# amd/aocl-sparse

Measured on AMD Instinct MI355X. Metric: CSR SpMV fp64 GFLOP/s + achieved-HBM-GB/s %roofline, higher is better.
Workload: dtype f64; 1 GPU; aoclsparse_dmv, 5-pt Laplacian grid 4096x4096 (m=16777216, nnz=83869696), alpha=1 beta=0; BASELINE configs[1] scaled past the 256 MiB Infinity Cache; parallelism=replicas x1, device=AMD Radeon Graphics (gfx950:sramecc+:...

## Files before the change

### aocl-sparse_amd/__init__.py

```python
import ctypes
import os
from ctypes import POINTER, byref, c_bool, c_char_p, c_double, c_float, c_int, c_int32, c_void_p

_HERE = os.path.dirname(os.path.abspath(__file__))
LIB_PATH = os.environ.get("AOCLSPARSE_MI355_LIB") or os.path.join(_HERE, "lib", "libaoclsparse_mi355.so")
INCLUDE_DIR = os.path.join(os.path.dirname(_HERE), "include")

OP_NONE, OP_TRANSPOSE, OP_CONJ_TRANSPOSE = 111, 112, 113
BASE_ZERO, BASE_ONE = 0, 1
TYPE_GENERAL, TYPE_SYMMETRIC, TYPE_HERMITIAN, TYPE_TRIANGULAR = 0, 1, 2, 3
DIAG_NON_UNIT, DIAG_UNIT, DIAG_ZERO = 0, 1, 2
FILL_LOWER, FILL_UPPER = 0, 1
ORDER_ROW, ORDER_COLUMN = 0, 1
STAGE_NNZ_COUNT, STAGE_FINALIZE, STAGE_FULL = 0, 1, 2
MEM_MINIMAL, MEM_UNRESTRICTED = 0, 1
PTR_AUTO, PTR_HOST, PTR_DEVICE = 0, 1, 2
OPTION_SPMV_KERNEL, OPTION_SELL, OPTION_SPMV_STRICT, OPTION_ALTERNATE_SWEEPS, OPTION_TRSV_CHUNKS = 0, 1, 2, 3, 4
OPTION_SELL_VALUES = 5
OPTION_ILU_SEARCH = 16
ILU_SEARCH_MIN = 21
COO_KEEP, COO_SUM = 0, 1
COO_KEEP_MAP = 16
COO_SORT_TILE = 4096
ORDER_SHORT_MAX = 32
ORDER_LDS_MAX = 2048
CLEAN_ROW_WAVE = 64

STATUS = {
    0: "success", 1: "not_implemented", 2: "invalid_pointer", 3: "invalid_size", 4: "internal_error",
    5: "invalid_value", 6: "invalid_index_value", 7: "maxit", 8: "user_stop", 9: "wrong_type",
    10: "memory_error", 11: "numerical_error", 12: "invalid_operation", 13: "unsorted_input",
    14: "invalid_kid",
}
# ... 414 lines not shown
    "aoclsparse_mi355_replicas_cloned": (c_int, [_P]),
    "aoclsparse_mi355_scsrmm_multi": (c_int, [c_int, c_float, _P, _P, c_int, _P, _I, _I, c_float, _P, _I, _I, _P]),
    "aoclsparse_mi355_dcsrmm_multi_slabs": (c_int, [c_int, c_double, _P, _P, c_int, _P, _I, _I, c_double, _P, _I, _I, _P]),
    "aoclsparse_mi355_scsrmm_shard": (c_int, [c_int, c_float, _P, _P, c_int, _P, _I, _I, c_float, _P, _I, _I, _I]),
    "aoclsparse_mi355_export_diag": (c_int, [_P, POINTER(_P), POINTER(_P), POINTER(_I)]),
    "aoclsparse_mi355_get_spmv_info": (c_int, [_P, c_int, POINTER(SpmvInfo)]),
    "aoclsparse_mi355_get_sell_values": (c_int, [_P, c_int, POINTER(_I)]),
    "aoclsparse_mi355_get_sell_packing": (c_int, [_P, c_int, POINTER(_I), POINTER(_I), POINTER(_I)]),
    "aoclsparse_mi355_get_sell_records": (c_int, [_P, c_int, POINTER(_I), POINTER(_I)]),
    "aoclsparse_mi355_get_sell_period": (c_int, [_P, c_int, POINTER(_I), POINTER(_I), POINTER(_I), POINTER(_I)]),
    "aoclsparse_mi355_sell_find_period": (c_int, [_I, _P, _P, _I, POINTER(_I), POINTER(ctypes.c_longlong)]),
    "aoclsparse_mi355_get_sell_march": (c_int, [_P, c_int, POINTER(_I), POINTER(_I), POINTER(_I), POINTER(_I)]),
    "aoclsparse_mi355_get_sell_keep_info": (c_int, [_P, c_int, _P]),
    "aoclsparse_mi355_sell_find_march": (c_int, [_I, _P, _P, POINTER(_I), _I, POINTER(_I)]),
    "aoclsparse_mi355_sell_march_rule": (c_int, [_I, _I, POINTER(_I), _I, _I, _I, _I, POINTER(_I)]),
    "aoclsparse_mi355_get_trsv_levels": (c_int, [_P, c_int, c_int, POINTER(_I)]),
    "aoclsparse_mi355_get_trsv_info": (c_int, [_P, c_int, c_int, POINTER(TrsvInfo)]),
    "aoclsparse_mi355_trsv_status": (c_int, [_P]),
    "aoclsparse_mi355_set_trsv_schedule": (c_int, [_I]),
    "aoclsparse_mi355_set_csrmm_beta0_overwrite": (c_int, [c_int]),
    "aoclsparse_mi355_invalidate": (c_int, [_P]),
    "aoclsparse_mi355_release_staging": (c_int, [POINTER(ctypes.c_size_t)]),
    "mi355_csrmv_plan_bound": (_I, [_I, _I]),
    "mi355_csrmv_plan_host": (_I, [_I, _I, _I, _P, _P]),
    "mi355_sell_slice_records": (_I, [_I, _P, _P, ctypes.c_longlong, _P]),
    "mi355_dcsrmv": (c_int, [_P, _I, _I, _I, _I, c_double, _I, _P, _P, _P, _P, _I, _P, c_double, _P]),
    "mi355_scsrmv": (c_int, [_P, _I, _I, _I, _I, c_float, _I, _P, _P, _P, _P, _I, _P, c_float, _P]),
    "mi355_dcsrmm": (c_int, [_P, _I, _I, c_double, _I, _I, _P, _P, _P, _P, _I, _I, c_double, _P, _I]),
}

# ... 268 lines not shown
    def sell_packing(self, op=OP_NONE):
        b, w, u = _I(-1), _I(-1), _I(-1)
        assert lib().aoclsparse_mi355_get_sell_packing(self.h, op, byref(b), byref(w), byref(u)) == 0
        return b.value, w.value, u.value

    def sell_records(self, op=OP_NONE):
        u, e = _I(-1), _I(-1)
        assert lib().aoclsparse_mi355_get_sell_records(self.h, op, byref(u), byref(e)) == 0
        return u.value, e.value

    def sell_period(self, op=OP_NONE):
        a, b, p, c = _I(-1), _I(-1), _I(-1), _I(-1)
        assert lib().aoclsparse_mi355_get_sell_period(self.h, op, byref(a), byref(b), byref(p), byref(c)) == 0
        return a.value, b.value, p.value, c.value

    def sell_march(self, op=OP_NONE):
        a, b, g, c = _I(-1), _I(-1), _I(-1), _I(-1)
        assert lib().aoclsparse_mi355_get_sell_march(self.h, op, byref(a), byref(b), byref(g), byref(c)) == 0
        return a.value, b.value, g.value, c.value

    def sell_keep_info(self, op=OP_NONE):
        info = SellKeepInfo(struct_size=ctypes.sizeof(SellKeepInfo))
        st = lib().aoclsparse_mi355_get_sell_keep_info(self.h, op, byref(info))
        assert st == 0, STATUS.get(st, st)
        return info

    def trsv_info(self, fill, op=OP_NONE):
        info = TrsvInfo()
        assert lib().aoclsparse_mi355_get_trsv_info(self.h, fill, op, byref(info)) == 0
        return info
# ... 167 lines not shown
    assert records.ndim == 2 and records.shape[1] == 4 and lists.shape == (records.shape[0], 8)
    out = (_I * 2)(-1, -1)
    st = lib().aoclsparse_mi355_sell_find_march(records.shape[0], _ptr(records), _ptr(lists), (_I * 4)(*rng), word_bytes, out)
    assert st == 0, STATUS.get(st, st)
    return tuple(out)


def sell_march_rule(nslices, max_width, rng, stack, alias_map, value_bytes=8, slices_per_wavefront=2):
    out = (_I * 4)(-1, -1, -1, -1)
    st = lib().aoclsparse_mi355_sell_march_rule(nslices, max_width, (_I * 4)(*rng), stack, alias_map, value_bytes,
                                                slices_per_wavefront, out)
    assert st == 0, STATUS.get(st, st)
    return tuple(out)


def device_info():
    dev, cus = c_int32(-1), c_int32(0)
    name = ctypes.create_string_buffer(256)
    st = lib().aoclsparse_mi355_device_info(byref(dev), byref(cus), name)
    return st, dev.value, cus.value, name.value.decode()


def hip_runtime_path():
    buf = ctypes.create_string_buffer(4096)
    st = lib().aoclsparse_mi355_hip_runtime_path(buf, 4096)
    return st, buf.value.decode()


def timer_start():
    return lib().aoclsparse_mi355_timer_start()
# ... 48 lines not shown
```

### aocl-sparse_amd/csrc/internal.hpp

```cpp
#pragma once

#include "aoclsparse.h"
#include "aoclsparse_mi355.h"

#include <hip/hip_runtime_api.h>

#include <atomic>
#include <algorithm>
#include <thread>
#include <cstdlib>
#include <cstdio>
#include <chrono>
#include <cstddef>
#include <cstdint>
#include <cstdint>
#include <exception>
#include <memory>
#include <mutex>
#include <functional>
#include <new>
#include <shared_mutex>
#include <system_error>
#include <vector>

// ... 1235 lines not shown
aoclsparse_status launch_roti(hipStream_t s, aoclsparse_int nnz, T *x, const aoclsparse_int *indx, T *y, T c, T sn);
template <typename T>
aoclsparse_status launch_doti(hipStream_t s, aoclsparse_int nnz, const T *x, const aoclsparse_int *indx, const T *y,
                              bool conj, T *partial, T *out);

template <typename T>
aoclsparse_status launch_sorv_level(hipStream_t s, const aoclsparse_int *rows, aoclsparse_int count, int base,
                                    const aoclsparse_int *ptr, const aoclsparse_int *ind, const T *val, T omega, T *x,
                                    const T *xold, const T *b);

constexpr int SPMV_TREE_MIN = 32;
constexpr int spmv_maxrows(int tile)
{
    return tile / 2 < 512 ? tile / 2 : 512;
}

}
```

### aocl-sparse_amd/csrc/matrix.cpp

```cpp
#include "spg_host.hpp"

#include <algorithm>
#include <atomic>
#include <climits>
#include <cstdlib>
#include <cstring>
#include <numeric>
#include <thread>

using namespace mi355;

namespace mi355
{

doid get_doid(const _aoclsparse_mat_descr *d, aoclsparse_operation op)
{
    const bool tr = op != aoclsparse_operation_none;
    switch(d->type)
    {
    case aoclsparse_matrix_type_general:
        return tr ? doid::gt : doid::gn;
    case aoclsparse_matrix_type_symmetric:
    case aoclsparse_matrix_type_hermitian:
        return d->fill_mode == aoclsparse_fill_mode_lower ? doid::sl : doid::su;
// ... 446 lines not shown
    }
    blocks[2 * nb]     = m;
    blocks[2 * nb + 1] = row_ptr[m] - base;
    if(long_rows)
        *long_rows = lr;
    if(max_row)
        *max_row = mx;
    return nb;
}

static aoclsparse_int choose_tile(aoclsparse_int , aoclsparse_int nnz, size_t vsize)
{
    if(vsize == 4 && (long long)nnz >= 1024LL * 256 * 16)
        return 2048;
    static const bool xcd_order = getenv("AOCLSPARSE_MI355_SPMV_XCD_ORDER") && getenv("AOCLSPARSE_MI355_SPMV_XCD_ORDER")[0] == '1';
    return ((long long)nnz < 1024LL * 256 * 16 ? 512 : 1024) | (xcd_order ? 1 : 0);
}

static void plan_rows_range(aoclsparse_int r0, aoclsparse_int r1, aoclsparse_index_base base, aoclsparse_int tile,
                            const aoclsparse_int *row_ptr, std::vector<aoclsparse_int> &out, aoclsparse_int &lr,
                            aoclsparse_int &mx)
{
    aoclsparse_int i = r0;
    while(i < r1)
    {
        const aoclsparse_int start = row_ptr[i] - base;
        aoclsparse_int       j     = i;
        while(j < r1 && j - i < spmv_maxrows(tile) && (row_ptr[j + 1] - base) - start <= tile)
            j++;
        if(j == i)
// ... 1292 lines not shown
```

### aocl-sparse_amd/csrc/runtime.cpp

```cpp
#include "internal.hpp"

#include <dlfcn.h>
#include <sys/mman.h>

#include <cctype>
#include <condition_variable>
#include <cstdio>
#include <cstdlib>
#include <cstring>
#include <thread>

#include <sched.h>

namespace mi355
{

aoclsparse_status map_hip_error(hipError_t e)
{
    if(e == hipSuccess)
        return aoclsparse_status_success;
    (void)hipGetLastError();
    if(e == hipErrorOutOfMemory)
        return aoclsparse_status_memory_error;
    return aoclsparse_status_internal_error;
// ... 275 lines not shown
}

std::atomic<bool> &csrmm_beta0_overwrite_flag()
{
    static std::atomic<bool> flag{[] {
        const char *e = std::getenv("AOCLSPARSE_MI355_CSRMM_BETA0_OVERWRITE");
        return e && std::atoi(e) != 0;
    }()};
    return flag;
}

namespace
{
    std::atomic<int> g_plan_options[aoclsparse_mi355_option_count] = {{0}, {-1}, {0}, {1}, {-1}, {-1}};
    std::atomic<int> g_ilu_search{-1};
}
unsigned long long stream_uid(hipStream_t s)
{
    using get_id_t = hipError_t (*)(hipStream_t, unsigned long long *);
    static const get_id_t get_id = [] {
        Dl_info info;
        if(!dladdr(reinterpret_cast<const void *>(&hipStreamCreate), &info) || !info.dli_fname)
            return static_cast<get_id_t>(nullptr);
        void *h = dlopen(info.dli_fname, RTLD_LAZY | RTLD_NOLOAD);
        return h ? reinterpret_cast<get_id_t>(dlsym(h, "hipStreamGetId")) : static_cast<get_id_t>(nullptr);
    }();
    unsigned long long id = 0;
    if(!get_id)
        return 0;
    if(get_id(s, &id) != hipSuccess)
    {
        (void)hipGetLastError();
        id = 0;
    }
    return id;
}

int plan_option(aoclsparse_mi355_option option)
{
    if(option == aoclsparse_mi355_option_ilu_search)
        return g_ilu_search.load(std::memory_order_relaxed);
    return option >= 0 && option < aoclsparse_mi355_option_count ? g_plan_options[option].load(std::memory_order_relaxed) : 0;
}

bool csrmm_reads_c(bool beta_nonzero)
{
    return beta_nonzero || !csrmm_beta0_overwrite_flag().load(std::memory_order_relaxed);
}

bool Runtime::is_device_pointer(const void *p)
{
    if(tl_device_scope > 0)
        return true;
    if(pointer_mode == aoclsparse_mi355_pointer_device)
        return true;
    if(pointer_mode == aoclsparse_mi355_pointer_host)
// ... 70 lines not shown
        if(scope.status == aoclsparse_status_success)
            f += r->release_staging();
    }
    if(bytes_freed)
        *bytes_freed = f;
    return aoclsparse_status_success;
}

aoclsparse_status aoclsparse_mi355_set_option(aoclsparse_mi355_option option, aoclsparse_int value)
{
    if(option == aoclsparse_mi355_option_ilu_search)
    {
        if(value < -1 || value > 1)
            return aoclsparse_status_invalid_value;
        g_ilu_search.store((int)value, std::memory_order_relaxed);
        return aoclsparse_status_success;
    }
    if(option < 0 || option >= aoclsparse_mi355_option_count)
        return aoclsparse_status_invalid_value;
    if(option == aoclsparse_mi355_option_spmv_kernel && (value < 0 || value > 2))
        return aoclsparse_status_invalid_value;
    if(option == aoclsparse_mi355_option_sell && (value < -1 || value > 1))
        return aoclsparse_status_invalid_value;
    if(option == aoclsparse_mi355_option_spmv_strict && (value < 0 || value > 1))
        return aoclsparse_status_invalid_value;
    if(option == aoclsparse_mi355_option_alternate_sweeps && (value < 0 || value > 1))
        return aoclsparse_status_invalid_value;
    if(option == aoclsparse_mi355_option_trsv_chunks && (value < -1 || value > 1))
        return aoclsparse_status_invalid_value;
    if(option == aoclsparse_mi355_option_sell_values && (value < -1 || value > 1))
// ... 181 lines not shown
```

### aocl-sparse_amd/csrc/spmv_api.cpp

```cpp
#include "internal.hpp"

#include <algorithm>
#include <cstring>
#include <vector>

using namespace mi355;

namespace
{

inline bool valid_op(aoclsparse_operation op)
{
    return op == aoclsparse_operation_none || op == aoclsparse_operation_transpose
           || op == aoclsparse_operation_conjugate_transpose;
}
inline bool valid_base(int b)
{
    return b == aoclsparse_index_base_zero || b == aoclsparse_index_base_one;
}
inline bool valid_type(int t)
{
    return t >= aoclsparse_matrix_type_general && t <= aoclsparse_matrix_type_triangular;
}

// ... 238 lines not shown
        }
    }
    std::shared_lock<std::shared_mutex> r(A->guard);
    return run_on_device_csr<T>(cs, kid, *dcsr, *plan, *alpha, x, *beta, y, dcsr->n, dcsr->m);
}

struct RawPlan
{
    const void               *key = nullptr;
    aoclsparse_int            m = -1, nnz = -1, base = -1;
    std::shared_ptr<SpmvPlan> plan;
};
constexpr int RAW_CACHE = 8;
RawPlan       g_raw[RAW_CACHE];
int           g_raw_next = 0;

template <typename T>
aoclsparse_status csrmv_t(aoclsparse_operation trans, const T *alpha, aoclsparse_int m,
                          aoclsparse_int n, aoclsparse_int nnz, const T *val,
                          const aoclsparse_int *col, const aoclsparse_int *row,
                          const aoclsparse_mat_descr descr, const T *x, const T *beta, T *y,
                          aoclsparse_matrix_data_type vt)
{
    if(!alpha || !beta)
        return aoclsparse_status_invalid_pointer;
    if(!descr)
        return aoclsparse_status_invalid_pointer;
    if(!valid_base(descr->base))
        return aoclsparse_status_invalid_value;
    if(!valid_type(descr->type))
// ... 153 lines not shown
                        held = e.plan;
            }
            if(rt.plan_stale_host && *rt.plan_stale_host)
            {
                std::lock_guard<std::mutex> g(rt.lock);
                *rt.plan_stale_host = 0;
                for(auto &e : g_raw)
                    e = RawPlan();
                held.reset();
            }
            if(held && !rt.plan_stale_dev)
                held.reset();
            if(!held)
            {
                fresh_plan = true;
                std::vector<aoclsparse_int> hrow((size_t)m + 1);
                MI355_HIP_TRY(hipMemcpy(hrow.data(), row, sizeof(aoclsparse_int) * ((size_t)m + 1),
                                        hipMemcpyDeviceToHost));
                held = std::make_shared<SpmvPlan>();
                st   = build_spmv_plan(m, nnz, descr->base, hrow.data(), *held, sizeof(T));
                if(st != aoclsparse_status_success)
                    return st;
                std::lock_guard<std::mutex> g(rt.lock);
                RawPlan                    *slot = nullptr;
                for(auto &e : g_raw)
                    if(e.key == row && e.m == m && e.nnz == nnz && e.base == descr->base)
                        slot = &e;
                if(!slot)
                {
                    slot       = &g_raw[g_raw_next];
// ... 154 lines not shown
            break;
        }
    int  order  = 0;
    bool strict = false;
    if(A->val_type == aoclsparse_smat)
        resolve_order<float>(kid, d.m, d.nnz, p.max_row_nnz, order, strict);
    else
        resolve_order<double>(kid, d.m, d.nnz, p.max_row_nnz, order, strict);
    info->order = order;
    if(plan_option(aoclsparse_mi355_option_spmv_strict) == 1)
        strict = true;
    info->tree_min = ((info->kernel == 1 || info->kernel == 2) && order == 0 && !strict) ? SPMV_TREE_MIN : 0;
    return aoclsparse_status_success;
}

aoclsparse_status aoclsparse_mi355_get_sell_values(const aoclsparse_matrix A, aoclsparse_operation op, aoclsparse_int *table_entries)
{
    if(!A || !table_entries)
        return aoclsparse_status_invalid_pointer;
    std::shared_lock<std::shared_mutex> r(A->guard);
    const SpmvPlan                     &p = op != aoclsparse_operation_none ? A->plan_trans : A->plan_user;
    *table_entries                        = p.sell.valid ? p.sell.ntab : 0;
    return aoclsparse_status_success;
}

aoclsparse_status aoclsparse_mi355_get_sell_packing(const aoclsparse_matrix A, aoclsparse_operation op, aoclsparse_int *index_bits,
                                                    aoclsparse_int *word_bytes, aoclsparse_int *uniform_slices)
{
    if(!A || !index_bits || !word_bytes || !uniform_slices)
        return aoclsparse_status_invalid_pointer;
// ... 110 lines not shown
```

### aocl-sparse_amd/csrc/spmv_kernels.hip

```cpp
#include "internal.hpp"

#include <hip/hip_runtime.h>

#include <cstdio>
#include <cstdlib>
#include <vector>

#include <algorithm>

namespace mi355
{

__device__ __forceinline__ double dev_fma(double a, double b, double c)
{
    return fma(a, b, c);
}
__device__ __forceinline__ float dev_fma(float a, float b, float c)
{
    return fmaf(a, b, c);
}

template <typename T>
__device__ __forceinline__ T finish(T r, T alpha, T beta, const T *yi)
{
// ... 91 lines not shown
__device__ __forceinline__ float read_lane(float v, int lane)
{
    return __int_as_float(__builtin_amdgcn_readlane(__float_as_int(v), lane));
}
template <typename T>
__device__ __forceinline__ T wave_sum(T v)
{
    v += dpp_mov<0xB1>(v);
    v += dpp_mov<0x4E>(v);
    v += dpp_mov<0x141>(v);
    v += dpp_mov<0x140>(v);
    return (read_lane(v, 0) + read_lane(v, 16)) + (read_lane(v, 32) + read_lane(v, 48));
}

constexpr int TREE_MIN = SPMV_TREE_MIN;

template <typename T, int ORDER, int TILE, int BLOCK, bool TRACE = false, int VAR = 0>
__global__ __launch_bounds__(BLOCK) void csr_adaptive_kernel(const int2 *__restrict__ blocks,
                                                                  const aoclsparse_int *__restrict__ row_ptr,
                                                                  const aoclsparse_int *__restrict__ col,
                                                                  const T *__restrict__ val,
                                                                  const T *__restrict__ x,
                                                                  T *__restrict__ y,
                                                                  T   alpha,
                                                                  T   beta,
                                                                  int base,
                                                                  int nblocks,
                                                                  int chunk,
                                                                  int flags,
                                                                  unsigned long long *trace,
// ... 102 lines not shown
                    s_x[i]   = xb[col[w0 + i]];
                }
            }
        }
        if constexpr(TRACE)
            t_st[2] = __builtin_amdgcn_s_memrealtime();
        __syncthreads();
        if constexpr(TRACE)
            t_st[3] = __builtin_amdgcn_s_memrealtime();
        const int grp  = tid / L;
        const int lane = tid % L;
        if((flags & 32) && (s_row[0] + w0 != p0 || s_row[nrows] + w0 != p0 + cnt))
        {
            if(tid == 0)
                __hip_atomic_store(stale, 1u, __ATOMIC_RELAXED, __HIP_MEMORY_SCOPE_SYSTEM);
            for(int rr = grp; rr < nrows; rr += BLOCK / L)
            {
                const int s = s_row[rr] + w0, e = s_row[rr + 1] + w0, r = r0 + rr;
                T         acc = T(0);
                if constexpr(L == 1)
                {
                    for(int j = s; j < e; j++)
                        acc = dev_fma(val[j], xb[col[j]], acc);
                    y[r] = finish(acc, alpha, beta, &y[r]);
                }
                else
                {
                    const int nfull = (e - s) & ~(L - 1);
                    for(int j = s + lane; j < s + nfull; j += L)
                        acc = dev_fma(val[j], xb[col[j]], acc);
                    T res = group_reduce<T, ORDER>(acc);
                    if(lane == 0)
                    {
                        if(nfull == 0)
                            res = T(0);
                        for(int j = s + nfull; j < e; j++)
                            res = dev_fma(val[j], xb[col[j]], res);
                        y[r] = finish(res, alpha, beta, &y[r]);
                    }
                }
            }
            return;
        }
        if constexpr(L == 1 && VAR == 0)
        {
            const int lane64 = tid & 63;
            for(int rb = 0; rb < nrows; rb += BLOCK)
            {
                const int  rr  = rb + tid;
                const bool act = rr < nrows;
                int        s = 0, e = 0;
                if(act)
                    s = s_row[rr], e = s_row[rr + 1];
                const bool lng = e - s >= TREE_MIN;
                if(act && !lng)
                {
// ... 47 lines not shown
                }
            }
        }
        else
        for(int rr = grp; rr < nrows; rr += BLOCK / L)
        {
            const int s   = s_row[rr];
            const int e   = s_row[rr + 1];
            const int r   = r0 + rr;
            T         acc = T(0);
            if constexpr(L == 1)
            {
                int j = s;
                if constexpr(VAR == 2)
                {
                    for(; j < e; j++)
                        acc = dev_fma(s_val[j], s_x[j], acc);
                }
                else
                {
                if(e - j >= 9)
                {
                    if(j & 1)
                    {
                        acc = dev_fma(s_val[j], s_x[j], acc);
                        j++;
                    }
                    P2   a[4], b[4], an[4], bn[4];
                    auto rd = [&](P2(&va)[4], P2(&vb)[4], int at) {
#pragma unroll
                        for(int q = 0; q < 4; q++)
                        {
// ... 172 lines not shown
            }
            for(; j < n; j += BLOCK)
                acc = dev_fma(val[p0 + j], xb[col[p0 + j]], acc);
            T res = block_sum<T, BLOCK>(acc, s_val);
            if(tid == 0)
                y[r0] = finish(res, alpha, beta, &y[r0]);
        }
    }
    if(TRACE && tid == 0)
    {
        unsigned long long *tr = trace + 8 * (size_t)b;
        tr[0] = t_st[0], tr[1] = t_st[1], tr[2] = t_st[2], tr[3] = t_st[3], tr[4] = __builtin_amdgcn_s_memrealtime();
        tr[5] = ((unsigned long long)(unsigned)nrows << 32) | (unsigned)cnt;
        tr[6] = (unsigned long long)r0, tr[7] = 0;
    }
}

template <typename T>
__global__ void scale_kernel(T *y, aoclsparse_int n, T beta)
{
    const int i = blockIdx.x * blockDim.x + threadIdx.x;
    if(i < n)
        y[i] = beta != T(0) ? beta * y[i] : T(0);
}

template <typename T>
__global__ void gather_strided_kernel(const T *src, aoclsparse_int inc, aoclsparse_int n, T *dst)
{
    const int i = blockIdx.x * blockDim.x + threadIdx.x;
    if(i < n)
// ... 39 lines not shown
    __syncthreads();
    if(threadIdx.x == 0)
        *d = (sh[0] + sh[1]) + (sh[2] + sh[3]);
}

template <typename T>
aoclsparse_status launch_dot(hipStream_t s, aoclsparse_int n, const T *x, const T *y, T *partial, T *d)
{
    const int blocks = n <= 0 ? 1 : (int)std::min<long long>(DOT_BLOCKS, ((long long)n + 255) / 256);
    hipLaunchKernelGGL((dot_partial_kernel<T>), dim3(blocks), dim3(256), 0, s, x, y, n, partial);
    hipLaunchKernelGGL((dot_final_kernel<T>), dim3(1), dim3(256), 0, s, partial, blocks, d);
    MI355_HIP_TRY(hipGetLastError());
    return aoclsparse_status_success;
}

template <typename T, int ORDER, int TILE, int BLOCK, int VAR>
static void launch_inst(hipStream_t s, int flags, int base, T alpha, const T *val, const aoclsparse_int *col,
                        const aoclsparse_int *row_ptr, const aoclsparse_int *blocks, aoclsparse_int nblocks,
                        const T *x, T beta, T *y, const aoclsparse_int *blocks4, unsigned int *stale)
{
    const int chunk = (nblocks + 7) / 8;
    const int grid  = (flags & 4) ? chunk * 8 : (int)nblocks;
    static const char  *trace_path = getenv("AOCLSPARSE_MI355_SPMV_TRACE");
    unsigned long long *trace      = nullptr;
    if(trace_path && hipMalloc(&trace, sizeof(unsigned long long) * 8 * (size_t)nblocks) != hipSuccess)
        trace = nullptr;
    if constexpr(ORDER == 0)
    {
        if(trace)
            hipLaunchKernelGGL((csr_adaptive_kernel<T, ORDER, TILE, BLOCK, true, VAR>), dim3(grid), dim3(BLOCK), 0, s,
                               reinterpret_cast<const int2 *>(blocks), row_ptr, col, val, x, y, alpha, beta, base,
                               (int)nblocks, chunk, flags, trace, reinterpret_cast<const int4 *>(blocks4), stale);
    }
    else if(trace)
    {
        (void)hipFree(trace);
        trace = nullptr;
    }
// ... 29 lines not shown
    int flags = strict ? 1 : 0;
    if(reinterpret_cast<uintptr_t>(val) % 16 == 0 && reinterpret_cast<uintptr_t>(col) % 16 == 0)
        flags |= 2;
    if(xcd)
        flags |= 4;
    if((size_t)m * sizeof(T) > (size_t)32 << 20)
        flags |= 8;
    const int var = strict ? 1 : (max_row_nnz <= 8 ? 2 : 0);
    if(stale)
        flags |= 32;
    if(rev && !xcd)
        flags |= 64;
    const int tsel = tile == 512 ? 0 : (tile == 1024 ? 1 : (tile == 2048 ? 2 : -1));
    if(tsel < 0 || order < 0 || order > 2)
        return aoclsparse_status_invalid_kid;
#define MI355_CASE(O, TL, BL)                                                                                                \
    if(var == 1)                                                                                                             \
        launch_inst<T, O, TL, BL, 1>(s, flags, base, alpha, val, col, row_ptr, blocks, nblocks, x, beta, y, blocks4, stale); \
    else if(var == 2)                                                                                                        \
        launch_inst<T, O, TL, BL, 2>(s, flags, base, alpha, val, col, row_ptr, blocks, nblocks, x, beta, y, blocks4, stale); \
    else                                                                                                                     \
        launch_inst<T, O, TL, BL, 0>(s, flags, base, alpha, val, col, row_ptr, blocks, nblocks, x, beta, y, blocks4, stale); \
    break
    switch(order * 3 + tsel)
    {
    case 0:
        MI355_CASE(0, 512, 128);
    case 1:
        MI355_CASE(0, 1024, 256);
    case 2:
// ... 125 lines not shown
```

### include/aoclsparse_mi355.h

```cpp
#ifndef AOCLSPARSE_MI355_H_
#define AOCLSPARSE_MI355_H_

#include "aoclsparse.h"

#include <stddef.h>

#ifdef __cplusplus
extern "C" {
#endif

typedef enum aoclsparse_mi355_pointer_mode_
{
    aoclsparse_mi355_pointer_auto   = 0,
    aoclsparse_mi355_pointer_host   = 1,
    aoclsparse_mi355_pointer_device = 2
} aoclsparse_mi355_pointer_mode;

DLL_PUBLIC aoclsparse_status aoclsparse_mi355_set_pointer_mode(aoclsparse_mi355_pointer_mode mode);
typedef enum aoclsparse_mi355_option_
{
    aoclsparse_mi355_option_spmv_kernel = 0,
    aoclsparse_mi355_option_sell        = 1,
    aoclsparse_mi355_option_spmv_strict = 2,
    aoclsparse_mi355_option_alternate_sweeps = 3,
    aoclsparse_mi355_option_trsv_chunks = 4,
    aoclsparse_mi355_option_sell_values = 5,
    aoclsparse_mi355_option_count       = 6,
    aoclsparse_mi355_option_ilu_search  = 16
} aoclsparse_mi355_option;
#define AOCLSPARSE_MI355_ILU_SEARCH_MIN 21
DLL_PUBLIC aoclsparse_status aoclsparse_mi355_set_option(aoclsparse_mi355_option option, aoclsparse_int value);
DLL_PUBLIC aoclsparse_status aoclsparse_mi355_set_csrmm_beta0_overwrite(int overwrite);
DLL_PUBLIC aoclsparse_status aoclsparse_mi355_set_stream(void *hip_stream);
DLL_PUBLIC void             *aoclsparse_mi355_get_stream(void);
DLL_PUBLIC aoclsparse_status aoclsparse_mi355_synchronize(void);
DLL_PUBLIC aoclsparse_status aoclsparse_mi355_device_info(aoclsparse_int *device,
                                                          aoclsparse_int *compute_units,
                                                          char            name[256]);
DLL_PUBLIC aoclsparse_status aoclsparse_mi355_hip_runtime_path(char *path, size_t capacity);
DLL_PUBLIC aoclsparse_status aoclsparse_mi355_timer_start(void);
DLL_PUBLIC aoclsparse_status aoclsparse_mi355_timer_stop(float *elapsed_ms);
DLL_PUBLIC aoclsparse_status aoclsparse_mi355_timer_mark(void);
DLL_PUBLIC aoclsparse_status aoclsparse_mi355_timer_laps(float *laps_ms, aoclsparse_int capacity, aoclsparse_int *count);

// ... 203 lines not shown
DLL_PUBLIC aoclsparse_status aoclsparse_mi355_get_sell_packing(const aoclsparse_matrix A, aoclsparse_operation op,
                                                               aoclsparse_int *index_bits, aoclsparse_int *word_bytes,
                                                               aoclsparse_int *uniform_slices);
DLL_PUBLIC aoclsparse_status aoclsparse_mi355_get_sell_records(const aoclsparse_matrix A, aoclsparse_operation op,
                                                               aoclsparse_int *uniform_word_slices,
                                                               aoclsparse_int *exception_slices);
DLL_PUBLIC aoclsparse_status aoclsparse_mi355_get_sell_period(const aoclsparse_matrix A, aoclsparse_operation op,
                                                              aoclsparse_int *first_slice, aoclsparse_int *end_slice,
                                                              aoclsparse_int *period_slices, aoclsparse_int *column_stride);
DLL_PUBLIC aoclsparse_status aoclsparse_mi355_sell_find_period(aoclsparse_int nslices, const void *records,
                                                               const aoclsparse_int *lists, aoclsparse_int max_period,
                                                               aoclsparse_int range[4], long long *comparisons);
DLL_PUBLIC aoclsparse_status aoclsparse_mi355_get_sell_march(const aoclsparse_matrix A, aoclsparse_operation op,
                                                             aoclsparse_int *first_slice, aoclsparse_int *end_slice,
                                                             aoclsparse_int *periods, aoclsparse_int *alias_map);
typedef struct
{
    size_t         struct_size;
    aoclsparse_int kept;
    aoclsparse_int valid;
    aoclsparse_int last_route;
    aoclsparse_int reserved;
    long long      structure_builds;
    long long      value_fills;
    long long      searches_skipped;
    long long      kept_bytes;
} aoclsparse_mi355_sell_keep_info;
DLL_PUBLIC aoclsparse_status aoclsparse_mi355_get_sell_keep_info(const aoclsparse_matrix A, aoclsparse_operation op,
                                                                 aoclsparse_mi355_sell_keep_info *info);
DLL_PUBLIC aoclsparse_status aoclsparse_mi355_sell_find_march(aoclsparse_int nslices, const void *records,
// ... 110 lines not shown
```

Baseline: 3720 GFLOP/s.

## Add multi-block streaming CSR SpMV kernel with software-pipelined loads for short rows

```diff
diff --git a/aocl-sparse_amd/__init__.py b/aocl-sparse_amd/__init__.py
--- a/aocl-sparse_amd/__init__.py
+++ b/aocl-sparse_amd/__init__.py
@@ -17,6 +17,8 @@
 PTR_AUTO, PTR_HOST, PTR_DEVICE = 0, 1, 2
 OPTION_SPMV_KERNEL, OPTION_SELL, OPTION_SPMV_STRICT, OPTION_ALTERNATE_SWEEPS, OPTION_TRSV_CHUNKS = 0, 1, 2, 3, 4
 OPTION_SELL_VALUES = 5
+OPTION_CSR_STREAM = 18
+CSR_STREAM_G, CSR_STREAM_MIN_BLOCKS = 3, 43000
 OPTION_ILU_SEARCH = 16
 ILU_SEARCH_MIN = 21
 COO_KEEP, COO_SUM = 0, 1
@@ -461,6 +463,9 @@
     "aoclsparse_mi355_get_sell_keep_info": (c_int, [_P, c_int, _P]),
     "aoclsparse_mi355_sell_find_march": (c_int, [_I, _P, _P, POINTER(_I), _I, POINTER(_I)]),
     "aoclsparse_mi355_sell_march_rule": (c_int, [_I, _I, POINTER(_I), _I, _I, _I, _I, POINTER(_I)]),
+    "aoclsparse_mi355_get_csr_stream": (c_int, [_P, c_int, POINTER(_I)]),
+    "aoclsparse_mi355_get_raw_plan_builds": (c_int, [POINTER(ctypes.c_longlong)]),
+    "aoclsparse_mi355_csr_stream_rule": (c_int, [_I, _I, _I, _I, _I, _I, _I, _I, POINTER(_I)]),
     "aoclsparse_mi355_get_trsv_levels": (c_int, [_P, c_int, c_int, POINTER(_I)]),
     "aoclsparse_mi355_get_trsv_info": (c_int, [_P, c_int, c_int, POINTER(TrsvInfo)]),
     "aoclsparse_mi355_trsv_status": (c_int, [_P]),
@@ -759,6 +764,11 @@
         assert lib().aoclsparse_mi355_get_sell_period(self.h, op, byref(a), byref(b), byref(p), byref(c)) == 0
         return a.value, b.value, p.value, c.value
 
+    def csr_stream(self, op=OP_NONE):
+        g = _I(-1)
+        assert lib().aoclsparse_mi355_get_csr_stream(self.h, op, byref(g)) == 0
+        return g.value
+
     def sell_march(self, op=OP_NONE):
         a, b, g, c = _I(-1), _I(-1), _I(-1), _I(-1)
         assert lib().aoclsparse_mi355_get_sell_march(self.h, op, byref(a), byref(b), byref(g), byref(c)) == 0
@@ -956,6 +966,19 @@
     return tuple(out)
 
 
+def csr_stream_rule(nblocks, max_row_nnz, order=0, strict=0, tile_word=1024, value_bytes=8, heavy_first=0, option=-1):
+    g = _I(-1)
+    st = lib().aoclsparse_mi355_csr_stream_rule(nblocks, max_row_nnz, order, strict, tile_word, value_bytes, heavy_first, option, byref(g))
+    assert st == 0, STATUS.get(st, st)
+    return g.value
+
+
+def raw_plan_builds():
+    n = ctypes.c_longlong(-1)
+    assert lib().aoclsparse_mi355_get_raw_plan_builds(byref(n)) == 0
+    return n.value
+
+
 def device_info():
     dev, cus = c_int32(-1), c_int32(0)
     name = ctypes.create_string_buffer(256)
diff --git a/aocl-sparse_amd/csrc/internal.hpp b/aocl-sparse_amd/csrc/internal.hpp
--- a/aocl-sparse_amd/csrc/internal.hpp
+++ b/aocl-sparse_amd/csrc/internal.hpp
@@ -1273,5 +1273,17 @@
 {
     return tile / 2 < 512 ? tile / 2 : 512;
 }
-
-}
+constexpr int CSR_STREAM_G = AOCLSPARSE_MI355_CSR_STREAM_G, CSR_STREAM_MIN_BLOCKS = AOCLSPARSE_MI355_CSR_STREAM_MIN_BLOCKS;
+inline int csr_stream_rule(aoclsparse_int nblocks, aoclsparse_int max_row_nnz, int order, bool strict, int tile_word, size_t vsize,
+                           bool blocks4, int option)
+{
+    if(option == 0 || nblocks <= 0 || max_row_nnz > 8 || order != 0 || strict || (tile_word & ~2) != 1024 || blocks4
+       || (vsize != 8 && vsize != 4))
+        return 0;
+    if(option >= 2 && option <= 4)
+        return option;
+    return nblocks >= CSR_STREAM_MIN_BLOCKS ? CSR_STREAM_G : 0;
+}
+bool spmv_traced();
+
+}
diff --git a/aocl-sparse_amd/csrc/matrix.cpp b/aocl-sparse_amd/csrc/matrix.cpp
--- a/aocl-sparse_amd/csrc/matrix.cpp
+++ b/aocl-sparse_amd/csrc/matrix.cpp
@@ -484,6 +484,8 @@
     if(vsize == 4 && (long long)nnz >= 1024LL * 256 * 16)
         return 2048;
     static const bool xcd_order = getenv("AOCLSPARSE_MI355_SPMV_XCD_ORDER") && getenv("AOCLSPARSE_MI355_SPMV_XCD_ORDER")[0] == '1';
+    if(const int forced = plan_option(aoclsparse_mi355_option_csr_stream); forced >= 2 && forced <= 4)
+        return 1024 | (xcd_order ? 1 : 0);
     return ((long long)nnz < 1024LL * 256 * 16 ? 512 : 1024) | (xcd_order ? 1 : 0);
 }
 
diff --git a/aocl-sparse_amd/csrc/runtime.cpp b/aocl-sparse_amd/csrc/runtime.cpp
--- a/aocl-sparse_amd/csrc/runtime.cpp
+++ b/aocl-sparse_amd/csrc/runtime.cpp
@@ -313,6 +313,7 @@
 {
     std::atomic<int> g_plan_options[aoclsparse_mi355_option_count] = {{0}, {-1}, {0}, {1}, {-1}, {-1}};
     std::atomic<int> g_ilu_search{-1};
+    std::atomic<int> g_csr_stream{-1};
 }
 unsigned long long stream_uid(hipStream_t s)
 {
@@ -339,6 +340,8 @@
 {
     if(option == aoclsparse_mi355_option_ilu_search)
         return g_ilu_search.load(std::memory_order_relaxed);
+    if(option == aoclsparse_mi355_option_csr_stream)
+        return g_csr_stream.load(std::memory_order_relaxed);
     return option >= 0 && option < aoclsparse_mi355_option_count ? g_plan_options[option].load(std::memory_order_relaxed) : 0;
 }
 
@@ -439,6 +442,13 @@
         if(value < -1 || value > 1)
             return aoclsparse_status_invalid_value;
         g_ilu_search.store((int)value, std::memory_order_relaxed);
+        return aoclsparse_status_success;
+    }
+    if(option == aoclsparse_mi355_option_csr_stream)
+    {
+        if(value != -1 && value != 0 && (value < 2 || value > 4))
+            return aoclsparse_status_invalid_value;
+        g_csr_stream.store((int)value, std::memory_order_relaxed);
         return aoclsparse_status_success;
     }
     if(option < 0 || option >= aoclsparse_mi355_option_count)
diff --git a/aocl-sparse_amd/csrc/spmv_api.cpp b/aocl-sparse_amd/csrc/spmv_api.cpp
--- a/aocl-sparse_amd/csrc/spmv_api.cpp
+++ b/aocl-sparse_amd/csrc/spmv_api.cpp
@@ -276,6 +276,7 @@
 constexpr int RAW_CACHE = 8;
 RawPlan       g_raw[RAW_CACHE];
 int           g_raw_next = 0;
+std::atomic<long long> g_raw_builds{0};
 
 template <typename T>
 aoclsparse_status csrmv_t(aoclsparse_operation trans, const T *alpha, aoclsparse_int m,
@@ -459,6 +460,7 @@
             if(!held)
             {
                 fresh_plan = true;
+                g_raw_builds.fetch_add(1, std::memory_order_relaxed);
                 std::vector<aoclsparse_int> hrow((size_t)m + 1);
                 MI355_HIP_TRY(hipMemcpy(hrow.data(), row, sizeof(aoclsparse_int) * ((size_t)m + 1),
                                         hipMemcpyDeviceToHost));
@@ -643,6 +645,59 @@
     return aoclsparse_status_success;
 }
 
+aoclsparse_status aoclsparse_mi355_get_csr_stream(const aoclsparse_matrix A, aoclsparse_operation op, aoclsparse_int *blocks_per_workgroup)
+{
+    if(!A || !blocks_per_workgroup)
+        return aoclsparse_status_invalid_pointer;
+    *blocks_per_workgroup = 0;
+    std::shared_lock<std::shared_mutex> r(A->guard);
+    const bool                          tr = op != aoclsparse_operation_none;
+    const SpmvPlan                     &p  = tr ? A->plan_trans : A->plan_user;
+    const DeviceCsr                    &d  = tr ? A->dev_trans : A->dev_user;
+    if(A->input_format == aoclsparse_bsr_mat || A->input_format == aoclsparse_tcsr_mat || is_complex_type(A->val_type) || !p.valid
+       || p.sell.valid)
+        return aoclsparse_status_success;
+    aoclsparse_int kid = -1;
+    for(const Hint &h : A->hints)
+        if(h.act == action_mv && h.id == (tr ? doid::gt : doid::gn))
+        {
+            kid = h.kid;
+            break;
+        }
+    int  order  = 0;
+    bool strict = false;
+    if((A->val_type == aoclsparse_smat ? resolve_order<float>(kid, d.m, d.nnz, p.max_row_nnz, order, strict)
+                                       : resolve_order<double>(kid, d.m, d.nnz, p.max_row_nnz, order, strict))
+       != aoclsparse_status_success)
+        return aoclsparse_status_success;
+    if(plan_option(aoclsparse_mi355_option_spmv_strict) == 1)
+        strict = true;
+    if((p.merge.valid && order == 0 && !strict) || spmv_traced())
+        return aoclsparse_status_success;
+    *blocks_per_workgroup = csr_stream_rule(p.nblocks, p.max_row_nnz, order, strict, p.tile, val_size(A->val_type),
+                                            p.heavy_first && (p.tile & 1) == 0, plan_option(aoclsparse_mi355_option_csr_stream));
+    return aoclsparse_status_success;
+}
+
+aoclsparse_status aoclsparse_mi355_get_raw_plan_builds(long long *builds)
+{
+    if(!builds)
+        return aoclsparse_status_invalid_pointer;
+    *builds = g_raw_builds.load(std::memory_order_relaxed);
+    return aoclsparse_status_success;
+}
+
+aoclsparse_status aoclsparse_mi355_csr_stream_rule(aoclsparse_int nblocks, aoclsparse_int max_row_nnz, aoclsparse_int order,
+                                                   aoclsparse_int strict, aoclsparse_int tile_word, aoclsparse_int value_bytes,
+                                                   aoclsparse_int heavy_first, aoclsparse_int option, aoclsparse_int *blocks_per_workgroup)
+{
+    if(!blocks_per_workgroup)
+        return aoclsparse_status_invalid_pointer;
+    *blocks_per_workgroup = csr_stream_rule(nblocks, max_row_nnz, (int)order, strict != 0, (int)tile_word, (size_t)value_bytes,
+                                            heavy_first != 0, (int)option);
+    return aoclsparse_status_success;
+}
+
 aoclsparse_status aoclsparse_mi355_get_sell_values(const aoclsparse_matrix A, aoclsparse_operation op, aoclsparse_int *table_entries)
 {
     if(!A || !table_entries)
diff --git a/aocl-sparse_amd/csrc/spmv_kernels.hip b/aocl-sparse_amd/csrc/spmv_kernels.hip
--- a/aocl-sparse_amd/csrc/spmv_kernels.hip
+++ b/aocl-sparse_amd/csrc/spmv_kernels.hip
@@ -4,6 +4,7 @@
 
 #include <cstdio>
 #include <cstdlib>
+#include <type_traits>
 #include <vector>
 
 #include <algorithm>
@@ -129,6 +130,50 @@
 }
 
 constexpr int TREE_MIN = SPMV_TREE_MIN;
+
+template <typename T, int ORDER, int BLOCK>
+__device__ __forceinline__ void live_rows(const aoclsparse_int *s_row, int w0, int r0, int nrows, const aoclsparse_int *__restrict__ col,
+                                          const T *__restrict__ val, const T *xb, T *__restrict__ y, T alpha, T beta)
+{
+    constexpr int L    = lanes_of<ORDER>::value;
+    const int     grp  = threadIdx.x / L;
+    const int     lane = threadIdx.x % L;
+    for(int rr = grp; rr < nrows; rr += BLOCK / L)
+    {
+        const int s = s_row[rr] + w0, e = s_row[rr + 1] + w0, r = r0 + rr;
+        T         acc = T(0);
+        if constexpr(L == 1)
+        {
+            for(int j = s; j < e; j++)
+                acc = dev_fma(val[j], xb[col[j]], acc);
+            y[r] = finish(acc, alpha, beta, &y[r]);
+        }
+        else
+        {
+            const int nfull = (e - s) & ~(L - 1);
+            for(int j = s + lane; j < s + nfull; j += L)
+                acc = dev_fma(val[j], xb[col[j]], acc);
+            T res = group_reduce<T, ORDER>(acc);
+            if(lane == 0)
+            {
+                if(nfull == 0)
+                    res = T(0);
+                for(int j = s + nfull; j < e; j++)
+                    res = dev_fma(val[j], xb[col[j]], res);
+                y[r] = finish(res, alpha, beta, &y[r]);
+            }
+        }
+    }
+}
+
+template <typename T>
+__device__ __forceinline__ T short_row_chain(const T *s_val, const T *s_x, int s, int e)
+{
+    T acc = T(0);
+    for(int j = s; j < e; j++)
+        acc = dev_fma(s_val[j], s_x[j], acc);
+    return acc;
+}
 
 template <typename T, int ORDER, int TILE, int BLOCK, bool TRACE = false, int VAR = 0>
 __global__ __launch_bounds__(BLOCK) void csr_adaptive_kernel(const int2 *__restrict__ blocks,
@@ -261,32 +306,7 @@
         {
             if(tid == 0)
                 __hip_atomic_store(stale, 1u, __ATOMIC_RELAXED, __HIP_MEMORY_SCOPE_SYSTEM);
-            for(int rr = grp; rr < nrows; rr += BLOCK / L)
-            {
-                const int s = s_row[rr] + w0, e = s_row[rr + 1] + w0, r = r0 + rr;
-                T         acc = T(0);
-                if constexpr(L == 1)
-                {
-                    for(int j = s; j < e; j++)
-                        acc = dev_fma(val[j], xb[col[j]], acc);
-                    y[r] = finish(acc, alpha, beta, &y[r]);
-                }
-                else
-                {
-                    const int nfull = (e - s) & ~(L - 1);
-                    for(int j = s + lane; j < s + nfull; j += L)
-                        acc = dev_fma(val[j], xb[col[j]], acc);
-                    T res = group_reduce<T, ORDER>(acc);
-                    if(lane == 0)
-                    {
-                        if(nfull == 0)
-                            res = T(0);
-                        for(int j = s + nfull; j < e; j++)
-                            res = dev_fma(val[j], xb[col[j]], res);
-                        y[r] = finish(res, alpha, beta, &y[r]);
-                    }
-                }
-            }
+            live_rows<T, ORDER, BLOCK>(s_row, w0, r0, nrows, col, val, xb, y, alpha, beta);
             return;
         }
         if constexpr(L == 1 && VAR == 0)
@@ -364,8 +384,7 @@
                 int j = s;
                 if constexpr(VAR == 2)
                 {
-                    for(; j < e; j++)
-                        acc = dev_fma(s_val[j], s_x[j], acc);
+                    acc = short_row_chain<T>(s_val, s_x, s, e);
                 }
                 else
                 {
@@ -568,6 +587,298 @@
         tr[5] = ((unsigned long long)(unsigned)nrows << 32) | (unsigned)cnt;
         tr[6] = (unsigned long long)r0, tr[7] = 0;
     }
+}
+
+template <typename T>
+struct StreamSet
+{
+    aoclsparse_int c0, c1, c2, c3, ct, rp0, rp1, rp2;
+    T              v0, v1, v2, v3, vt;
+};
+struct StreamBlock
+{
+    int r0, p0, nrows, cnt, w0, cntw;
+};
+struct StreamLane
+{
+    bool quad, e0, e1, e2, e3, tail;
+    int  rem;
+};
+template <int BLOCK>
+__device__ __forceinline__ StreamLane stream_lane(const StreamBlock &k, int flags)
+{
+    const int  tid = threadIdx.x;
+    const bool al  = (flags & 2) != 0;
+    StreamLane l;
+    l.quad = al && 4 * tid + 3 < k.cntw;
+    l.e0   = !al && tid < k.cntw;
+    l.e1   = !al && tid + BLOCK < k.cntw;
+    l.e2   = !al && tid + 2 * BLOCK < k.cntw;
+    l.e3   = !al && tid + 3 * BLOCK < k.cntw;
+    l.rem  = (k.cntw & ~3) + tid;
+    l.tail = al && tid < 3 && l.rem < k.cntw;
+    return l;
+}
+
+template <typename T, int TILE, int BLOCK>
+__device__ __forceinline__ void stream_load(StreamSet<T> &s, const StreamBlock &k, const aoclsparse_int *__restrict__ row_ptr,
+                                            const aoclsparse_int *__restrict__ col, const T *__restrict__ val, int flags)
+{
+    using P2           = typename pair_of<T>::type;
+    const int        tid = threadIdx.x;
+    const StreamLane l   = stream_lane<BLOCK>(k, flags);
+    if(tid <= k.nrows)
+        s.rp0 = row_ptr[k.r0 + tid];
+    if(tid + BLOCK <= k.nrows)
+        s.rp1 = row_ptr[k.r0 + tid + BLOCK];
+    if(tid + 2 * BLOCK <= k.nrows)
+        s.rp2 = row_ptr[k.r0 + tid + 2 * BLOCK];
+    if(l.quad)
+    {
+        const int  i = k.w0 + 4 * tid;
+        const int4 c = *reinterpret_cast<const int4 *>(col + i);
+        s.c0 = c.x, s.c1 = c.y, s.c2 = c.z, s.c3 = c.w;
+        if constexpr(sizeof(T) == 8)
+        {
+            const P2 va = *reinterpret_cast<const P2 *>(val + i);
+            const P2 vb = *reinterpret_cast<const P2 *>(val + i + 2);
+            s.v0 = va.x, s.v1 = va.y, s.v2 = vb.x, s.v3 = vb.y;
+        }
+        else
+        {
+            const float4 vq = *reinterpret_cast<const float4 *>(val + i);
+            s.v0 = vq.x, s.v1 = vq.y, s.v2 = vq.z, s.v3 = vq.w;
+        }
+    }
+    if(l.tail)
+        s.ct = col[k.w0 + l.rem], s.vt = val[k.w0 + l.rem];
+    if(l.e0)
+        s.c0 = col[k.w0 + tid], s.v0 = val[k.w0 + tid];
+    if(l.e1)
+        s.c1 = col[k.w0 + tid + BLOCK], s.v1 = val[k.w0 + tid + BLOCK];
+    if(l.e2)
+        s.c2 = col[k.w0 + tid + 2 * BLOCK], s.v2 = val[k.w0 + tid + 2 * BLOCK];
+    if(l.e3)
+        s.c3 = col[k.w0 + tid + 3 * BLOCK], s.v3 = val[k.w0 + tid + 3 * BLOCK];
+}
+
+template <typename T>
+struct StreamX
+{
+    T x0, x1, x2, x3, xt;
+};
+template <typename T, int BLOCK>
+__device__ __forceinline__ void stream_gather(const StreamSet<T> &s, const StreamBlock &k, const T *xb, int flags, StreamX<T> &g)
+{
+    const StreamLane l = stream_lane<BLOCK>(k, flags);
+    if(l.quad || l.e0)
+        g.x0 = xb[s.c0];
+    if(l.quad || l.e1)
+        g.x1 = xb[s.c1];
+    if(l.quad || l.e2)
+        g.x2 = xb[s.c2];
+    if(l.quad || l.e3)
+        g.x3 = xb[s.c3];
+    if(l.tail)
+        g.xt = xb[s.ct];
+}
+
+template <typename T, int BLOCK>
+__device__ __forceinline__ void stream_fill(const StreamSet<T> &s, const StreamX<T> &g, const StreamBlock &k, int base, int flags,
+                                            T *s_val, T *s_x, aoclsparse_int *s_row)
+{
+    const int        tid = threadIdx.x;
+    const StreamLane l   = stream_lane<BLOCK>(k, flags);
+    if(tid <= k.nrows)
+        s_row[tid] = s.rp0 - base - k.w0;
+    if(tid + BLOCK <= k.nrows)
+        s_row[tid + BLOCK] = s.rp1 - base - k.w0;
+    if(tid + 2 * BLOCK <= k.nrows)
+        s_row[tid + 2 * BLOCK] = s.rp2 - base - k.w0;
+    if(l.quad)
+    {
+        const int i  = 4 * tid;
+        s_val[i]     = s.v0;
+        s_val[i + 1] = s.v1;
+        s_val[i + 2] = s.v2;
+        s_val[i + 3] = s.v3;
+        s_x[i]       = g.x0;
+        s_x[i + 1]   = g.x1;
+        s_x[i + 2]   = g.x2;
+        s_x[i + 3]   = g.x3;
+    }
+    if(l.tail)
+        s_val[l.rem] = s.vt, s_x[l.rem] = g.xt;
+    if(l.e0)
+        s_val[tid] = s.v0, s_x[tid] = g.x0;
+    if(l.e1)
+        s_val[tid + BLOCK] = s.v1, s_x[tid + BLOCK] = g.x1;
+    if(l.e2)
+        s_val[tid + 2 * BLOCK] = s.v2, s_x[tid + 2 * BLOCK] = g.x2;
+    if(l.e3)
+        s_val[tid + 3 * BLOCK] = s.v3, s_x[tid + 3 * BLOCK] = g.x3;
+}
+
+template <int BLOCK>
+__device__ __forceinline__ int stream_quad_at(const StreamBlock &k)
+{
+    return min(4 * (int)threadIdx.x, (k.cntw - 4) & ~3);
+}
+__device__ __forceinline__ int stream_rem_at(const StreamBlock &k)
+{
+    return min((k.cntw & ~3) + (int)threadIdx.x, k.cntw - 1);
+}
+template <typename T, int BLOCK>
+__device__ __forceinline__ void stream_load_fast(StreamSet<T> &s, const StreamBlock &k, const aoclsparse_int *__restrict__ row_ptr,
+                                                 const aoclsparse_int *__restrict__ col, const T *__restrict__ val)
+{
+    using P2      = typename pair_of<T>::type;
+    const int tid = threadIdx.x;
+    s.rp0 = row_ptr[k.r0 + min(tid, k.nrows)];
+    s.rp1 = row_ptr[k.r0 + min(tid + BLOCK, k.nrows)];
+    s.rp2 = row_ptr[k.r0 + min(tid + 2 * BLOCK, k.nrows)];
+    const int  i = k.w0 + stream_quad_at<BLOCK>(k);
+    const int4 c = *reinterpret_cast<const int4 *>(col + i);
+    s.c0 = c.x, s.c1 = c.y, s.c2 = c.z, s.c3 = c.w;
+    if constexpr(sizeof(T) == 8)
+    {
+        const P2 va = *reinterpret_cast<const P2 *>(val + i);
+        const P2 vb = *reinterpret_cast<const P2 *>(val + i + 2);
+        s.v0 = va.x, s.v1 = va.y, s.v2 = vb.x, s.v3 = vb.y;
+    }
+    else
+    {
+        const float4 vq = *reinterpret_cast<const float4 *>(val + i);
+        s.v0 = vq.x, s.v1 = vq.y, s.v2 = vq.z, s.v3 = vq.w;
+    }
+    const int j = k.w0 + stream_rem_at(k);
+    s.ct = col[j], s.vt = val[j];
+}
+template <typename T>
+__device__ __forceinline__ void stream_gather_fast(const StreamSet<T> &s, const T *xb, StreamX<T> &g)
+{
+    g.x0 = xb[s.c0], g.x1 = xb[s.c1], g.x2 = xb[s.c2], g.x3 = xb[s.c3], g.xt = xb[s.ct];
+}
+template <typename T, int BLOCK>
+__device__ __forceinline__ void stream_fill_fast(const StreamSet<T> &s, const StreamX<T> &g, const StreamBlock &k, int base, T *s_val,
+                                                 T *s_x, aoclsparse_int *s_row)
+{
+    const int tid = threadIdx.x;
+    s_row[min(tid, k.nrows)]             = s.rp0 - base - k.w0;
+    s_row[min(tid + BLOCK, k.nrows)]     = s.rp1 - base - k.w0;
+    s_row[min(tid + 2 * BLOCK, k.nrows)] = s.rp2 - base - k.w0;
+    const int i  = stream_quad_at<BLOCK>(k);
+    s_val[i]     = s.v0;
+    s_val[i + 1] = s.v1;
+    s_val[i + 2] = s.v2;
+    s_val[i + 3] = s.v3;
+    s_x[i]       = g.x0;
+    s_x[i + 1]   = g.x1;
+    s_x[i + 2]   = g.x2;
+    s_x[i + 3]   = g.x3;
+    const int j = stream_rem_at(k);
+    s_val[j] = s.vt, s_x[j] = g.xt;
+}
+
+template <typename T, int TILE, int BLOCK, int G>
+__global__ __launch_bounds__(BLOCK) void csr_stream_kernel(const int2 *__restrict__ blocks,
+                                                                const aoclsparse_int *__restrict__ row_ptr,
+                                                                const aoclsparse_int *__restrict__ col,
+                                                                const T *__restrict__ val,
+                                                                const T *__restrict__ x,
+                                                                T *__restrict__ y,
+                                                                T   alpha,
+                                                                T   beta,
+                                                                int base,
+                                                                int nblocks,
+                                                                int flags,
+                                                                unsigned int *stale)
+{
+    static_assert(TILE == 4 * BLOCK && spmv_maxrows(TILE) + 1 <= 3 * BLOCK, "one quad per thread, <= 3 row_ptr words per thread");
+    constexpr int MAXROWS = spmv_maxrows(TILE);
+    __shared__ __attribute__((aligned(16))) T s_val[TILE + 4];
+    __shared__ __attribute__((aligned(16))) T s_x[TILE + 4];
+    __shared__ aoclsparse_int s_row[MAXROWS + 1];
+    const int tid = threadIdx.x;
+    const T  *xb  = x - base;
+    const int b0  = G * ((flags & 64) ? (int)gridDim.x - 1 - (int)blockIdx.x : (int)blockIdx.x);
+    int2 e[G + 1];
+#pragma unroll
+    for(int t = 0; t <= G; t++)
+        e[t] = blocks[min(b0 + t, nblocks)];
+    StreamBlock k[G];
+    bool        live[G];
+#pragma unroll
+    for(int t = 0; t < G; t++)
+    {
+        k[t].r0 = e[t].x, k[t].p0 = e[t].y, k[t].nrows = e[t + 1].x - e[t].x, k[t].cnt = e[t + 1].y - e[t].y;
+        k[t].w0   = (flags & 2) ? (k[t].p0 & ~3) : k[t].p0;
+        k[t].cntw = k[t].cnt + (k[t].p0 - k[t].w0);
+        live[t] = b0 + t < nblocks && k[t].cnt <= TILE;
+    }
+    bool fast = (flags & 2) != 0;
+#pragma unroll
+    for(int t = 0; t < G; t++)
+        fast = fast && live[t] && k[t].cntw >= 4;
+    StreamSet<T> sa, sb;
+    auto step = [&](auto fc, auto tc, StreamSet<T> &cur, StreamSet<T> &nxt) __attribute__((always_inline)) {
+        constexpr bool FAST = decltype(fc)::value;
+        constexpr int  t    = decltype(tc)::value;
+        StreamX<T>     xg;
+        if constexpr(FAST)
+            stream_gather_fast<T>(cur, xb, xg);
+        else if(live[t])
+            stream_gather<T, BLOCK>(cur, k[t], xb, flags, xg);
+        __builtin_amdgcn_sched_barrier(0);
+        if constexpr(t + 1 < G)
+        {
+            if constexpr(FAST)
+                stream_load_fast<T, BLOCK>(nxt, k[t + 1], row_ptr, col, val);
+            else if(live[t + 1])
+                stream_load<T, TILE, BLOCK>(nxt, k[t + 1], row_ptr, col, val, flags);
+        }
+        __builtin_amdgcn_sched_barrier(0);
+        if(!FAST && !live[t])
+            return;
+        if constexpr(t > 0)
+            __syncthreads();
+        if constexpr(FAST)
+            stream_fill_fast<T, BLOCK>(cur, xg, k[t], base, s_val, s_x, s_row);
+        else
+            stream_fill<T, BLOCK>(cur, xg, k[t], base, flags, s_val, s_x, s_row);
+        __syncthreads();
+        const int r0 = k[t].r0, nrows = k[t].nrows, w0 = k[t].w0;
+        if((flags & 32) && (s_row[0] + w0 != k[t].p0 || s_row[nrows] + w0 != k[t].p0 + k[t].cnt))
+        {
+            if(tid == 0)
+                __hip_atomic_store(stale, 1u, __ATOMIC_RELAXED, __HIP_MEMORY_SCOPE_SYSTEM);
+            live_rows<T, 0, BLOCK>(s_row, w0, r0, nrows, col, val, xb, y, alpha, beta);
+            return;
+        }
+        for(int rr = tid; rr < nrows; rr += BLOCK)
+        {
+            const int r   = r0 + rr;
+            const T   acc = short_row_chain<T>(s_val, s_x, s_row[rr], s_row[rr + 1]);
+            store_y(&y[r], finish(acc, alpha, beta, &y[r]), flags);
+        }
+    };
+    static_assert(G >= 2 && G <= 4, "the steps are written out below");
+    auto group = [&](auto fc) __attribute__((always_inline)) {
+        if constexpr(decltype(fc)::value)
+            stream_load_fast<T, BLOCK>(sa, k[0], row_ptr, col, val);
+        else if(live[0])
+            stream_load<T, TILE, BLOCK>(sa, k[0], row_ptr, col, val, flags);
+        step(fc, std::integral_constant<int, 0>{}, sa, sb);
+        step(fc, std::integral_constant<int, 1>{}, sb, sa);
+        if constexpr(G > 2)
+            step(fc, std::integral_constant<int, 2>{}, sa, sb);
+        if constexpr(G > 3)
+            step(fc, std::integral_constant<int, 3>{}, sb, sa);
+    };
+    if(fast)
+        group(std::true_type{});
+    else
+        group(std::false_type{});
 }
 
 template <typename T>
@@ -637,6 +948,16 @@
     return aoclsparse_status_success;
 }
 
+static const char *spmv_trace_path()
+{
+    static const char *path = getenv("AOCLSPARSE_MI355_SPMV_TRACE");
+    return path;
+}
+bool spmv_traced()
+{
+    return spmv_trace_path() != nullptr;
+}
+
 template <typename T, int ORDER, int TILE, int BLOCK, int VAR>
 static void launch_inst(hipStream_t s, int flags, int base, T alpha, const T *val, const aoclsparse_int *col,
                         const aoclsparse_int *row_ptr, const aoclsparse_int *blocks, aoclsparse_int nblocks,
@@ -644,7 +965,7 @@
 {
     const int chunk = (nblocks + 7) / 8;
     const int grid  = (flags & 4) ? chunk * 8 : (int)nblocks;
-    static const char  *trace_path = getenv("AOCLSPARSE_MI355_SPMV_TRACE");
+    const char         *trace_path = spmv_trace_path();
     unsigned long long *trace      = nullptr;
     if(trace_path && hipMalloc(&trace, sizeof(unsigned long long) * 8 * (size_t)nblocks) != hipSuccess)
         trace = nullptr;
@@ -704,6 +1025,24 @@
     const int tsel = tile == 512 ? 0 : (tile == 1024 ? 1 : (tile == 2048 ? 2 : -1));
     if(tsel < 0 || order < 0 || order > 2)
         return aoclsparse_status_invalid_kid;
+    if(const int g = spmv_traced() ? 0
+                                   : csr_stream_rule(nblocks, max_row_nnz, order, strict, tile | (xcd ? 1 : 0), sizeof(T), blocks4 != nullptr,
+                                                     plan_option(aoclsparse_mi355_option_csr_stream)))
+    {
+        const int grid = (int)((nblocks + g - 1) / g);
+#define MI355_STREAM(GG)                                                                                                     \
+    hipLaunchKernelGGL((csr_stream_kernel<T, 1024, 256, GG>), dim3(grid), dim3(256), 0, s, reinterpret_cast<const int2 *>(blocks), \
+                       row_ptr, col, val, x, y, alpha, beta, base, (int)nblocks, flags, stale)
+        if(g == 2)
+            MI355_STREAM(2);
+        else if(g == 3)
+            MI355_STREAM(3);
+        else
+            MI355_STREAM(4);
+#undef MI355_STREAM
+        MI355_HIP_TRY(hipGetLastError());
+        return aoclsparse_status_success;
+    }
 #define MI355_CASE(O, TL, BL)                                                                                                \
     if(var == 1)                                                                                                             \
         launch_inst<T, O, TL, BL, 1>(s, flags, base, alpha, val, col, row_ptr, blocks, nblocks, x, beta, y, blocks4, stale); \
diff --git a/include/aoclsparse_mi355.h b/include/aoclsparse_mi355.h
--- a/include/aoclsparse_mi355.h
+++ b/include/aoclsparse_mi355.h
@@ -26,8 +26,11 @@
     aoclsparse_mi355_option_trsv_chunks = 4,
     aoclsparse_mi355_option_sell_values = 5,
     aoclsparse_mi355_option_count       = 6,
-    aoclsparse_mi355_option_ilu_search  = 16
+    aoclsparse_mi355_option_ilu_search  = 16,
+    aoclsparse_mi355_option_csr_stream  = 18
 } aoclsparse_mi355_option;
+#define AOCLSPARSE_MI355_CSR_STREAM_G 3
+#define AOCLSPARSE_MI355_CSR_STREAM_MIN_BLOCKS 43000
 #define AOCLSPARSE_MI355_ILU_SEARCH_MIN 21
 DLL_PUBLIC aoclsparse_status aoclsparse_mi355_set_option(aoclsparse_mi355_option option, aoclsparse_int value);
 DLL_PUBLIC aoclsparse_status aoclsparse_mi355_set_csrmm_beta0_overwrite(int overwrite);
@@ -261,6 +264,13 @@
 DLL_PUBLIC aoclsparse_status aoclsparse_mi355_get_sell_march(const aoclsparse_matrix A, aoclsparse_operation op,
                                                              aoclsparse_int *first_slice, aoclsparse_int *end_slice,
                                                              aoclsparse_int *periods, aoclsparse_int *alias_map);
+DLL_PUBLIC aoclsparse_status aoclsparse_mi355_get_csr_stream(const aoclsparse_matrix A, aoclsparse_operation op,
+                                                             aoclsparse_int *blocks_per_workgroup);
+DLL_PUBLIC aoclsparse_status aoclsparse_mi355_get_raw_plan_builds(long long *builds);
+DLL_PUBLIC aoclsparse_status aoclsparse_mi355_csr_stream_rule(aoclsparse_int nblocks, aoclsparse_int max_row_nnz, aoclsparse_int order,
+                                                              aoclsparse_int strict, aoclsparse_int tile_word, aoclsparse_int value_bytes,
+                                                              aoclsparse_int heavy_first, aoclsparse_int option,
+                                                              aoclsparse_int *blocks_per_workgroup);
 typedef struct
 {
     size_t         struct_size;
```

Result: no change. 3724 GFLOP/s (median of 3 runs) (+0.1%).
